# nianticlabs/mickey

Measured on AMD Instinct MI355X. Metric: image pairs/sec (540x720), higher is better.
Workload: dtype bf16

## Files before the change

include/mickey_hip_dev.h:

```cpp
#ifndef MICKEY_HIP_DEV_H
#define MICKEY_HIP_DEV_H

#ifdef __cplusplus
extern "C" {
#endif

int mk_gemm_set_tile(int mode);

int mk_attn_set_mode(int mode);

int mk_dev_mfma_sustained(float* scratch, int workgroups, int iters, int zero_operands, void* stream);

#ifdef __cplusplus
}
#endif
#endif
```

mickey_amd/_native.py:

```python
import ctypes
import os

import torch

from . import build as _build

MK_BF16, MK_F16, MK_F32 = 0, 1, 2
ACT_NONE, ACT_RELU, ACT_GELU = 0, 1, 2

_P, _I, _L, _F, _U = ctypes.c_void_p, ctypes.c_int, ctypes.c_longlong, ctypes.c_float, ctypes.c_ulonglong
_CODES = {"p": _P, "i": _I, "l": _L, "f": _F, "u": _U}

SIGNATURES = {
    "mk_version": ("i", ""),
    "mk_last_error": ("s", ""),
    "mk_preprocess_u8": ("i", "pliiipiip"),
    "mk_gemm": ("i", "pipippiiiiiiip"),
    "mk_gemm_grouped": ("i", "pilpilplpiliiiiiiip"),
    "mk_gemm_ls_residual": ("i", "pipipppiiiiip"),
    "mk_gemm_qkv": ("i", "pipippppiiiifip"),
    "mk_gemm_patch_embed": ("i", "pipipppiiiiip"),
    "mk_gemm_ls_residual_ln": ("i", "pipippppipppiiiiip"),
    "mk_gemm_patch_embed_ln": ("i", "pipipppppiiiiip"),
    "mk_cls_token_ln": ("i", "pppppiiiip"),
# ... 20 lines not shown
    "mk_conv_train_weight_planes": ("i", "piiippppp"),
    "mk_conv_wgrad_work_floats": ("l", "iiiii"),
    "mk_conv_wgrad": ("i", "ppippiiiiippppp"),
    "mk_gemm_grouped_split": ("i", "ppilpilplppiliiiiiffpp"),
    "mk_posenc_add": ("i", "ppppiiiiiip"),
    "mk_linattn_work_floats": ("l", "iiii"),
    "mk_linattn_kv": ("i", "pppiiiip"),
    "mk_linattn_apply": ("i", "pppiiiiiip"),
    "mk_linattn_kv_fused": ("i", "pilpilppiiiiip"),
    "mk_linattn_apply_fused": ("i", "pilpilppilppfpiliiiiip"),
    "mk_linattn_train_work_floats": ("l", "iiii"),
    "mk_linattn_train_fwd": ("i", "pllpllpllfpppiiiip"),
    "mk_linattn_train_bwd": ("i", "pllpllpllppfpppppiiiip"),
    "mk_train_rows_per_chunk": ("i", "i"),
    "mk_train_chunks": ("i", "i"),
    "mk_train_ln_steps": ("i", "i"),
    "mk_train_linear_fwd": ("i", "pliplipppipliiip"),
    "mk_train_linear_ln128_fwd": ("i", "pliplipppfplpppip"),
    "mk_train_linear_dgrad": ("i", "pllipppiplplipliiiip"),
    "mk_train_linear_wgrad": ("i", "pllipliplipliiiip"),
    "mk_train_tail": ("i", "plilplilpp"),
    "mk_train_ln128_fwd": ("i", "pppfplpppip"),
    "mk_train_ln128_bwd": ("i", "pppppplip"),
    "mk_train_headtail_chunk_rows": ("i", ""),
    "mk_train_headtail_chunks": ("i", "l"),
    "mk_train_headtail_fwd": ("i", "pppiiiiiififfp"),
    "mk_train_headtail_bwd": ("i", "ppppppppiiiiiffp"),
    "mk_train_desc_l2norm_fwd": ("i", "pppiiifp"),
    "mk_train_desc_l2norm_bwd": ("i", "ppppiiip"),
    "mk_train_bn_chunk_rows": ("i", ""),
    "mk_train_bn_chunks": ("i", "l"),
    "mk_train_bn_work_floats": ("l", "li"),
    "mk_train_bn_fwd": ("i", "plppplpppffpplpppiiiip"),
    "mk_train_bn_bwd": ("i", "plplpppppplplppfiiip"),
    "mk_optim_chunk_elems": ("i", ""),
    "mk_optim_chunks": ("l", "l"),
    "mk_optim_grad_stats": ("i", "pipipp"),
    "mk_optim_reduce": ("i", "pifpp"),
    "mk_optim_adam": ("i", "pipipp"),
    "mk_head_tails": ("i", "pppppppppppiiiiiiiififp"),
    "mk_dual_softmax_work_floats": ("l", "iiii"),
    "mk_dual_softmax": ("i", "ppppfifppppiiiip"),
    "mk_dual_softmax_split_work_floats": ("l", "iii"),
    "mk_dual_softmax_split": ("i", "ppppfifppppiiiip"),
    "mk_sinkhorn_work_floats": ("l", "iii"),
    "mk_sinkhorn": ("i", "ppppfippppiiiip"),
    "mk_dual_softmax_kf": ("i", "ppppfifppppiiiipip"),
    "mk_dual_softmax_split_kf": ("i", "ppppfifppppiiiipip"),
    "mk_sinkhorn_kf": ("i", "ppppfippppiiiipip"),
    "mk_dual_softmax_pairs": ("i", "ppppfifppppiiiippiip"),
    "mk_dual_softmax_split_pairs_work_floats": ("l", "iiiiii"),
    "mk_dual_softmax_split_pairs": ("i", "ppppfifppppiiiippiip"),
    "mk_sinkhorn_pairs": ("i", "ppppfippppiiiippiip"),
    "mk_dsc_split_planes_floats": ("l", "ii"),
    "mk_dsc_split_planes": ("i", "ppiiip"),
    "mk_dual_softmax_split_planes_work_floats": ("l", "iii"),
    "mk_dual_softmax_split_planes": ("i", "ppppfifppppiiippiip"),
    "mk_mutual_nn": ("i", "ppppiiip"),
    "mk_dual_softmax_train_work_floats": ("l", "iiii"),
    "mk_dual_softmax_train": ("i", "ppppfppppppiiiiip"),
    "mk_dual_softmax_bwd_work_floats": ("l", "iiii"),
    "mk_dual_softmax_bwd": ("i", "ppppfpppppppppiiiiip"),
    "mk_exprace_topk_work_bytes": ("l", "iiil"),
    "mk_exprace_topk_state_bytes": ("l", "ii"),
    "mk_exprace_topk": ("i", "ppuupppppiiliip"),
    "mk_counter_add": ("i", "pup"),
    "mk_gather_backproject": ("i", "ppppppppppppiiiiip"),
    "mk_gather_backproject_kf": ("i", "ppppppppppppiiiiipip"),
    "mk_gather_backproject_pairs": ("i", "ppppppppppppiiiiippiip"),
    "mk_gather_backproject_bwd": ("i", "ppppppppppiiiiip"),
    "mk_ransac_hypotheses": ("i", "pppppuupfppppiiilp"),
    "mk_refine_pose": ("i", "pppppfiipppppppiiiip"),
    "mk_pose_finalize": ("i", "ppppip"),
    "mk_train_ransac_masks": ("i", "pppppuupfiipppiiilp"),
    "mk_reinforce_scatter": ("i", "ppppiiilp"),
    "mk_train_tail_fwd": ("i", "pppppppiiiifiifpppp"),
    "mk_train_tail_bwd": ("i", "pppppppiiiifiifppppppp"),
    "mk_train_aggregate_fwd": ("i", "pppiiififfppppp"),
    "mk_train_aggregate_bwd": ("i", "ppiiipp"),
}

DEV_SIGNATURES = {
    "mk_gemm_set_tile": ("i", "i"),
    "mk_attn_set_mode": ("i", "i"),
    "mk_dev_mfma_sustained": ("i", "piiip"),
}

_lib = None
_missing = set()


class MickeyHipError(RuntimeError):
    pass


def lib_path():
    return os.environ.get("MICKEY_HIP_LIB", _build.lib_path())


def load():
    global _lib
    if _lib is not None:
        return _lib
    path = lib_path()
    if not os.path.exists(path):
        raise MickeyHipError("libmickey_hip.so not found at %s -- build it with `python -m mickey_amd.build` "
                             "(mickey_amd has no CPU/ATen fallback)" % path)
    lib = ctypes.CDLL(path)
    for name, (res, args) in list(SIGNATURES.items()) + list(DEV_SIGNATURES.items()):
        try:
            fn = getattr(lib, name)
        except AttributeError:
            _missing.add(name)
            continue
        fn.restype = ctypes.c_char_p if res == "s" else _CODES[res]
        fn.argtypes = [_CODES[c] for c in args]
    _lib = lib
    return lib


def exported_symbols():
    return list(SIGNATURES)


def missing_symbols():
    load()
    return sorted(_missing)


def ptr(t):
    if t is None:
        return None
    if not t.is_cuda:
        raise MickeyHipError("expected a device tensor")
    return t.data_ptr()


def stream():
    return torch.cuda.current_stream().cuda_stream


def dtype_code(dt):
    if dt == torch.bfloat16:
        return MK_BF16
    if dt == torch.float16:
        return MK_F16
    if dt == torch.float32:
        return MK_F32
    raise MickeyHipError("unsupported low-precision dtype %s" % dt)


def call(name, *args):
    lib = load()
    if name in _missing:
        raise MickeyHipError("libmickey_hip.so does not export %s (stale build?)" % name)
    rc = getattr(lib, name)(*args)
    if rc != 0:
        raise MickeyHipError("%s failed (%d): %s" % (name, rc, lib.mk_last_error().decode()))


def query(name, *args):
    return getattr(load(), name)(*args)
```

mickey_amd/csrc/mk_gemm.hip:

```cpp
#include "mk_gemm_common.hpp"

namespace mk {
namespace gemm {
namespace {

template <typename T, int AMODE, int WMF, bool SP = false>
__global__ __launch_bounds__(256, 1) void gemm_kernel(GemmParams p) {
  using V8 = typename Lp<T>::V8;
  constexpr int NWM = 2, NWN = 2;
  constexpr int NW = NWM * NWN, BM = NWM * WMF * 16, BN = NWN * 64;
  constexpr int AJ = BM / 8 / NW, WJ = BN / 8 / NW;
  constexpr int A_BYTES = BM * 128, STAGE_BYTES = (BM + BN) * 128;
  constexpr int NS = WMF == 2 ? 3 : 2;
  constexpr int PIECES = AJ + WJ;
  extern __shared__ __attribute__((aligned(16))) char smem[];

  const int tid = threadIdx.x;
  const int lane = tid & 63;
  const int wave = __builtin_amdgcn_readfirstlane(tid >> 6);
  const int wm = wave / NWN, wn = wave % NWN;
  const int g = blockIdx.y;
  const int ntm = (p.M + BM - 1) / BM, ntn = (p.N + BN - 1) / BN;
  const int nk = p.K / BK;
  const int fr = lane & 15, fg = lane >> 4;

  const int id = xcd_remap(blockIdx.x, ntm * ntn);
  const int m0 = (id / ntn) * BM, n0 = (id % ntn) * BN;
  Stager<T, AMODE, NW, AJ, WJ, SP> st;
  st.init(p, g, m0, n0, wave, lane);
  st.issue(p, smem, smem + A_BYTES, 0);
  if (NS == 3 && nk > 1) st.issue(p, smem + STAGE_BYTES, smem + STAGE_BYTES + A_BYTES, 1);
  float2* lnp = (float2*)(smem + NS * STAGE_BYTES);
  if (AMODE == A_DENSE && p.ln_stats && tid < 2 * BM) ln_params_to_lds<BM, 2 * BM>(p, m0, tid, lnp, p.ln_shift_out != nullptr && n0 == 0);
  f32x4 acc[WMF][4];
#pragma unroll
  for (int i = 0; i < WMF; ++i)
#pragma unroll
    for (int j = 0; j < 4; ++j) acc[i][j] = f32x4{0.f, 0.f, 0.f, 0.f};
  int cur = 0, nxt = NS - 1;
  for (int kt = 0; kt < nk; ++kt) {
    if (NS == 3 && kt + 1 < nk) asm volatile("s_waitcnt vmcnt(%0)" ::"n"(PIECES) : "memory");
    else asm volatile("s_waitcnt vmcnt(0)" ::: "memory");
    asm volatile("s_waitcnt lgkmcnt(0)" ::: "memory");
    __builtin_amdgcn_s_barrier();
    char* nA = smem + nxt * STAGE_BYTES;
    if (kt + NS - 1 < nk) st.issue(p, nA, nA + A_BYTES, kt + NS - 1);
    const char* sA = smem + cur * STAGE_BYTES;
    const char* sW = sA + A_BYTES;
    cur = cur + 1 == NS ? 0 : cur + 1;
    nxt = nxt + 1 == NS ? 0 : nxt + 1;
    if constexpr (SP) {
      V8 wf[2][4], xf[2][WMF];
#pragma unroll
      for (int ks = 0; ks < 2; ++ks) {
#pragma unroll
        for (int i = 0; i < 4; ++i) {
          const int rw = wn * 64 + i * 16 + fr;
          wf[ks][i] = *(const V8*)(sW + rw * 128 + swz8(rw, ks * 4 + fg) * 16);
        }
#pragma unroll
        for (int i = 0; i < WMF; ++i) {
          const int rx = wm * (WMF * 16) + i * 16 + fr;
          xf[ks][i] = *(const V8*)(sA + rx * 128 + swz8(rx, ks * 4 + fg) * 16);
        }
      }
#pragma unroll
      for (int pr = 0; pr < 3; ++pr) {
        if (pr == 2 && p.npass == 2) break;
#pragma unroll
        for (int mi = 0; mi < WMF; ++mi)
#pragma unroll
          for (int ni = 0; ni < 4; ++ni) acc[mi][ni] = Lp<T>::mma16(wf[pr == 1][ni], xf[pr == 2][mi], acc[mi][ni]);
      }
    } else {
#pragma unroll
      for (int ks = 0; ks < 2; ++ks) {
        V8 wf[4], xf[WMF];
#pragma unroll
        for (int i = 0; i < 4; ++i) {
          const int rw = wn * 64 + i * 16 + fr;
          wf[i] = *(const V8*)(sW + rw * 128 + swz8(rw, ks * 4 + fg) * 16);
        }
#pragma unroll
        for (int i = 0; i < WMF; ++i) {
          const int rx = wm * (WMF * 16) + i * 16 + fr;
          xf[i] = *(const V8*)(sA + rx * 128 + swz8(rx, ks * 4 + fg) * 16);
        }
#pragma unroll
        for (int mi = 0; mi < WMF; ++mi)
#pragma unroll
          for (int ni = 0; ni < 4; ++ni) acc[mi][ni] = Lp<T>::mma16(wf[ni], xf[mi], acc[mi][ni]);
      }
    }
  }
  epilogue<T, WMF>(p, acc, m0, n0, wm, wn, lane, g, lnp);
}

template <typename T, int AMODE, int WMF, bool SP = false>
int launch_small(const GemmParams& p, int groups, hipStream_t st) {
  constexpr int BM = 32 * WMF;
  constexpr int LDS = (WMF == 2 ? 3 : 2) * (BM + 128) * 128 + BM * 8;
  static bool attr_done = false;
  if (!attr_done) {
    hipError_t e = hipFuncSetAttribute((const void*)gemm_kernel<T, AMODE, WMF, SP>, hipFuncAttributeMaxDynamicSharedMemorySize, LDS);
    if (e != hipSuccess) {
      mk_set_error("gemm: cannot reserve %d B of LDS: %s", LDS, hipGetErrorString(e));
      return MK_ERR_LAUNCH;
    }
    attr_done = true;
  }
  const int ntm = (p.M + BM - 1) / BM, ntn = (p.N + 127) / 128;
  hipLaunchKernelGGL((gemm_kernel<T, AMODE, WMF, SP>), dim3(ntm * ntn, groups, 1), dim3(256), LDS, st, p);
  MK_CHECK_LAUNCH();
  return MK_OK;
}

int g_num_cus = 0;
int g_band_m = 0;
int g_half_rows = 1;
int g_schedule = 0;

template <int AMODE>
int launch(const GemmParams& p, int groups, int dtype, hipStream_t st) {
  const long long big_tiles = (long long)((p.M + 255) / 256) * ((p.N + 255) / 256) * groups;
  bool big = p.N >= 256 && big_tiles >= 192;
  const long long plmax = p.npass > 1 ? (long long)max(max(p.pl1[0], p.pl1[1]), max(p.pl2[0], p.pl2[1])) / 2 : 0;
  const bool k_ok = p.K >= 2 * BK && (long long)p.M * p.lda + plmax < (1ll << 31) && (long long)p.N * p.ldw < (1ll << 31) &&
                    (AMODE == A_DENSE || bordered_rows(p.M / (p.H * p.Wd), p.H, p.Wd) * (p.C1 > p.C2 ? p.C1 : p.C2) + plmax < (1ll << 31));
  const bool ln_fold = p.ln_stats || p.xh;
  if (dtype == MK_F32) {
    MK_CHECK_ARG(!ln_fold, "gemm: the folded-LayerNorm epilogues exist for 16-bit operands only");
    return launch_f32(p, groups, AMODE, st);
  }
  int sched = g_schedule;
  if (sched == 0) sched = (big && k_ok) ? 7 : 1;
  if (!k_ok) sched = 1;
  if (sched == 7) return launch_pp64(p, groups, dtype, AMODE, st, g_band_m);
  const long long small_tiles = (long long)((p.M + 127) / 128) * ((p.N + 127) / 128) * groups;
  const bool half_rows = g_schedule == 2 || (g_schedule != 1 && g_half_rows && small_tiles < 2 * num_cus() && p.M > 64);
  if (p.npass > 1)
    return half_rows ? launch_small<_Float16, AMODE, 2, true>(p, groups, st) : launch_small<_Float16, AMODE, 4, true>(p, groups, st);
  if (half_rows) return dtype == MK_BF16 ? launch_small<__bf16, AMODE, 2>(p, groups, st) : launch_small<_Float16, AMODE, 2>(p, groups, st);
  return dtype == MK_BF16 ? launch_small<__bf16, AMODE, 4>(p, groups, st) : launch_small<_Float16, AMODE, 4>(p, groups, st);
}

int check_common(const GemmParams& p, int dtype) {
  MK_CHECK_ARG(dtype == MK_BF16 || dtype == MK_F16 || dtype == MK_F32, "gemm: dtype must be MK_BF16, MK_F16 or MK_F32");
  MK_CHECK_ARG(p.M > 0 && p.N > 0 && p.K > 0, "gemm: empty problem M=%d N=%d K=%d", p.M, p.N, p.K);
  const int kt = dtype == MK_F32 ? KT<float> : BK;
  MK_CHECK_ARG(p.K % kt == 0, "gemm: K=%d must be a multiple of %d", p.K, kt);
  MK_CHECK_ARG(p.N % 4 == 0, "gemm: N=%d must be a multiple of 4", p.N);
  MK_CHECK_ARG(p.ldw % 8 == 0 && p.ldw >= p.K, "gemm: ldw=%d must be >= K and a multiple of 8", p.ldw);
  MK_CHECK_ARG(p.A && p.W, "gemm: null operand");
  return MK_OK;
}

}

int num_cus() {
  if (g_num_cus == 0) {
    int dev = 0, n = 0;
    if (hipGetDevice(&dev) != hipSuccess || hipDeviceGetAttribute(&n, hipDeviceAttributeMultiprocessorCount, dev) != hipSuccess || n <= 0)
      n = 256;
    g_num_cus = n;
  }
  return g_num_cus;
}

}
}

using namespace mk;
using namespace mk::gemm;

extern "C" {

int mk_gemm_set_tile(int mode) {
  if (mode >= 400 && mode < 464) {
    g_band_m = mode - 400;
    return MK_OK;
  }
  if (mode >= 464 && mode < 496) {
    g_band_m = -(mode - 464);
    return MK_OK;
  }
  if (mode == 500 || mode == 501) {
    g_half_rows = mode - 500;
    return MK_OK;
  }
  if (mode >= 600 && mode <= 602) {
    g_pp64_persist = mode - 600;
    return MK_OK;
  }
  MK_CHECK_ARG(mode == 0 || mode == 1 || mode == 2 || mode == 7,
               "mk_gemm_set_tile: unknown mode %d (0 automatic, 1 128x128, 2 64x128, 7 8-wave ping-pong)", mode);
  g_schedule = mode;
  return MK_OK;
}

int mk_gemm(const void* A, int lda, const void* W, int ldw, const float* bias, void* out, int ldc, int M, int N, int K,
            int act, int out_is_f32, int dtype, mk_stream_t stream) {
  GemmParams p = {};
  p.A = A; p.W = W; p.M = M; p.N = N; p.K = K; p.lda = lda; p.ldw = ldw;
  p.epi = MK_EPI_STORE; p.act = act; p.bias = bias; p.ldc = ldc;
  if (out_is_f32) p.out_f32 = (float*)out; else p.out_lp = out;
  if (int e = check_common(p, dtype)) return e;
  MK_CHECK_ARG(lda % 8 == 0 && lda >= K && ldc % 4 == 0 && ldc >= N && out, "mk_gemm: bad lda/ldc/out");
  return launch<A_DENSE>(p, 1, dtype, (hipStream_t)stream);
}

int mk_gemm_grouped(const void* A, int lda, long long strideA, const void* W, int ldw, long long strideW, const float* bias,
                    long long strideBias, void* out, int ldc, long long strideOut, int groups, int M, int N, int K, int act,
                    int out_is_f32, int dtype, mk_stream_t stream) {
  GemmParams p = {};
  p.A = A; p.W = W; p.M = M; p.N = N; p.K = K; p.lda = lda; p.ldw = ldw;
  p.strideA_g = strideA; p.strideW_g = strideW; p.strideBias_g = strideBias; p.strideOut_g = strideOut;
  p.epi = MK_EPI_STORE; p.act = act; p.bias = bias; p.ldc = ldc;
  if (out_is_f32) p.out_f32 = (float*)out; else p.out_lp = out;
  if (int e = check_common(p, dtype)) return e;
  MK_CHECK_ARG(groups > 0 && lda % 8 == 0 && lda >= K && ldc % 4 == 0 && ldc >= N && out, "mk_gemm_grouped: bad args");
  return launch<A_DENSE>(p, groups, dtype, (hipStream_t)stream);
}

int mk_gemm_ls_residual(const void* A, int lda, const void* W, int ldw, const float* bias, const float* gamma, float* x,
                        int ldx, int M, int N, int K, int dtype, mk_stream_t stream) {
  GemmParams p = {};
  p.A = A; p.W = W; p.M = M; p.N = N; p.K = K; p.lda = lda; p.ldw = ldw;
  p.epi = MK_EPI_LS_RESIDUAL; p.bias = bias; p.gamma = gamma; p.out_f32 = x; p.ldc = ldx;
  if (int e = check_common(p, dtype)) return e;
  MK_CHECK_ARG(bias && gamma && x && lda % 8 == 0 && lda >= K && ldx % 4 == 0 && ldx >= N, "mk_gemm_ls_residual: bad args");
  return launch<A_DENSE>(p, 1, dtype, (hipStream_t)stream);
}

int mk_gemm_qkv(const void* A, int lda, const void* W, int ldw, const float* bias, void* q, void* k, void* vt, int nimg,
                int ntok, int ntok_pad, int heads, float qscale, int dtype, mk_stream_t stream) {
  GemmParams p = {};
  const int D = heads * 64;
  p.A = A; p.W = W; p.M = nimg * ntok; p.N = 3 * D; p.K = D; p.lda = lda; p.ldw = ldw;
  p.epi = MK_EPI_QKV; p.bias = bias; p.q = q; p.k = k; p.vt = vt;
  p.ntok = ntok; p.ntok_pad = ntok_pad; p.heads = heads; p.qscale = qscale;
  if (int e = check_common(p, dtype)) return e;
  MK_CHECK_ARG(bias && q && k && vt && ntok_pad % 64 == 0 && ntok_pad >= ntok && lda % 8 == 0 && lda >= D, "mk_gemm_qkv: bad args");
  return launch<A_DENSE>(p, 1, dtype, (hipStream_t)stream);
}

int mk_gemm_patch_embed(const void* A, int lda, const void* W, int ldw, const float* bias, const float* pos, float* x,
                        int nimg, int npatch, int D, int K, int dtype, mk_stream_t stream) {
  GemmParams p = {};
  p.A = A; p.W = W; p.M = nimg * npatch; p.N = D; p.K = K; p.lda = lda; p.ldw = ldw;
  p.epi = MK_EPI_PATCH; p.bias = bias; p.pos = pos; p.npatch = npatch; p.out_f32 = x; p.ldc = D;
  if (int e = check_common(p, dtype)) return e;
  MK_CHECK_ARG(bias && pos && x && lda % 8 == 0 && lda >= K, "mk_gemm_patch_embed: bad args");
  return launch<A_DENSE>(p, 1, dtype, (hipStream_t)stream);
}


static int ln_consumer_args(GemmParams& p, const float* colsum, const float* stats, float eps, float* shift_out, const char* who) {
  MK_CHECK_ARG(colsum && stats && p.bias, "%s: colsum, stats and bias are required", who);
  MK_CHECK_ARG(p.lda == p.K, "%s: the normalised width is K: lda must equal K", who);
  p.ln_colsum = colsum; p.ln_stats = stats; p.ln_nslot = p.K / 64; p.ln_eps = eps; p.ln_shift_out = shift_out;
  return MK_OK;
}

int mk_gemm_ln(const void* A, int lda, const void* W, int ldw, const float* bias, const float* colsum, const float* stats,
               float eps, float* shift_out, void* out, int ldc, int M, int N, int K, int act, int dtype, mk_stream_t stream) {
  GemmParams p = {};
  p.A = A; p.W = W; p.M = M; p.N = N; p.K = K; p.lda = lda; p.ldw = ldw;
  p.epi = MK_EPI_STORE; p.act = act; p.bias = bias; p.ldc = ldc; p.out_lp = out;
  if (int e = check_common(p, dtype)) return e;
  MK_CHECK_ARG(lda % 8 == 0 && ldc % 4 == 0 && ldc >= N && out && (act == MK_ACT_NONE || act == MK_ACT_GELU), "mk_gemm_ln: bad args");
  if (int e = ln_consumer_args(p, colsum, stats, eps, shift_out, "mk_gemm_ln")) return e;
  return launch<A_DENSE>(p, 1, dtype, (hipStream_t)stream);
}

int mk_gemm_qkv_ln(const void* A, int lda, const void* W, int ldw, const float* bias, const float* colsum, const float* stats,
                   float eps, float* shift_out, void* q, void* k, void* vt, int nimg, int ntok, int ntok_pad, int heads,
                   float qscale, int dtype, mk_stream_t stream) {
  GemmParams p = {};
  const int D = heads * 64;
// ... 146 lines not shown
```

mickey_amd/csrc/mk_gemm_common.hpp:

```cpp
#pragma once
#include "mk_common.hpp"

namespace mk {
namespace gemm {

constexpr int BK = 64;
template <typename T> constexpr int EPC = 16 / (int)sizeof(T);
template <typename T> constexpr int KT = 128 / (int)sizeof(T);

enum AMode { A_DENSE = 0, A_CONV3 = 1 };

struct GemmParams {
  const void* A;
  const void* A2;
  const void* W;
  int M, N, K, lda, ldw;
  long long strideA_g, strideA2_g, strideW_g;
  int H, Wd, C1, C2;
  int bord_out;
  unsigned pl1[2], pl2[2];
  int npass;
  float acc_scale;
  void* out_lo;
  float plane_scale;
  int* sat_flag;
  int epi;
  int act;
  const float* bias;
  const float* gamma;
  long long strideBias_g;
  float* out_f32;
  void* out_lp;
  int ldc;
  long long strideOut_g;
  const void* resid_lp;
  long long strideResid_g;
  void* q;
  void* k;
  void* vt;
  int ntok, ntok_pad, heads;
  float qscale;
  const float* pos;
  int npatch;
  void* xh;
  void* xl;
  int ldxs;
  float* stats_out;
  int nslot_out;
  const float* ln_stats;
  const float* ln_colsum;
  int ln_nslot;
  float ln_eps;
  float* ln_shift_out;
  const float* ln_shift_in;
};

__device__ __forceinline__ void quad_stats(const f32x4& x, float& s, float& q) {
  s = x[0];
  s += x[1];
  s += x[2];
  s += x[3];
  q = __builtin_fmaf(x[0], x[0], 0.0f);
  q = __builtin_fmaf(x[1], x[1], q);
  q = __builtin_fmaf(x[2], x[2], q);
  q = __builtin_fmaf(x[3], x[3], q);
}

__device__ __forceinline__ float row16_sum(float v) {
#define MK_DPP_ADD(ctrl) v += __builtin_bit_cast(float, __builtin_amdgcn_update_dpp(0, __builtin_bit_cast(int, v), ctrl, 0xf, 0xf, true))
  MK_DPP_ADD(0xB1);
  MK_DPP_ADD(0x4E);
  MK_DPP_ADD(0x141);
  MK_DPP_ADD(0x140);
#undef MK_DPP_ADD
  return v;
}

typedef __attribute__((ext_vector_type(4))) unsigned u32x4;
struct LnRowLoads16 {
  u32x4 v[4];
  __device__ __forceinline__ void issue(const GemmParams& p, int m0, int tid) {
    const int wave = tid >> 6, lane = tid & 63;
    const long long last = (long long)p.M * 128 - 16;
#pragma unroll
    for (int j = 0; j < 4; ++j) {
      long long off = ((long long)(m0 + wave * 32 + j * 8) * 128) + lane * 16;
      off = off < last ? off : last;
      const char* a = (const char*)p.ln_stats + off;
      asm volatile("global_load_dwordx4 %0, %1, off" : "=v"(v[j]) : "v"(a) : "memory");
    }
  }
  template <int YOUNGER>
  __device__ __forceinline__ void finish(const GemmParams& p, int tid, float2* prm, int m0 = 0, bool publish = false) {
    asm volatile("s_waitcnt vmcnt(%4)" : "+v"(v[0]), "+v"(v[1]), "+v"(v[2]), "+v"(v[3]) : "n"(YOUNGER) : "memory");
    const int wave = tid >> 6, lane = tid & 63;
#pragma unroll
    for (int j = 0; j < 4; ++j) {
      const f32x4 f = __builtin_bit_cast(f32x4, v[j]);
      float s = f[0] + f[2], q = f[1] + f[3];
#define MK_DPP_ADD(x, ctrl) x += __builtin_bit_cast(float, __builtin_amdgcn_update_dpp(0, __builtin_bit_cast(int, x), ctrl, 0xf, 0xf, true))
      MK_DPP_ADD(s, 0xB1);  MK_DPP_ADD(q, 0xB1);
      MK_DPP_ADD(s, 0x4E);  MK_DPP_ADD(q, 0x4E);
      MK_DPP_ADD(s, 0x141); MK_DPP_ADD(q, 0x141);
#undef MK_DPP_ADD
      const double mean = (double)s * (1.0 / 1024.0);
      double var = (double)q * (1.0 / 1024.0) - mean * mean;
      var = var > 0.0 ? var : 0.0;
      const float rstd = 1.0f / sqrtf((float)var + p.ln_eps);
      if ((lane & 7) == 0) {
        const int r = wave * 32 + j * 8 + (lane >> 3);
        prm[r] = make_float2(rstd, -(float)mean * rstd);
        if (publish && m0 + r < p.M) p.ln_shift_out[m0 + r] = (float)mean;
      }
    }
  }
};

struct LnRowDma16 {
  template <int J0>
  __device__ __forceinline__ static void issue(const GemmParams& p, int m0, int wave, int lane, char* stage_lds) {
    const long long last = (long long)p.M * 128 - 16;
#pragma unroll
    for (int j = J0; j < J0 + 2; ++j) {
      const long long base = (long long)(m0 + wave * 32 + j * 8) * 128;
      long long off = base + lane * 16;
      off = off < last ? off : last;
      glds16_sv((const char*)p.ln_stats, (unsigned)off, stage_lds + (wave * 2 + (j - J0)) * 1024);
    }
  }
  template <int J0>
  __device__ __forceinline__ static void finish(const GemmParams& p, int wave, int lane, float2* prm, const char* stage_lds, int m0,
                                                bool publish) {
#pragma unroll
    for (int j = J0; j < J0 + 2; ++j) {
      const f32x4 f = *(const f32x4*)(stage_lds + (wave * 2 + (j - J0)) * 1024 + lane * 16);
      float s = f[0] + f[2], q = f[1] + f[3];
#define MK_DPP_ADD(x, ctrl) x += __builtin_bit_cast(float, __builtin_amdgcn_update_dpp(0, __builtin_bit_cast(int, x), ctrl, 0xf, 0xf, true))
// ... 762 lines not shown
```

mickey_amd/csrc/mk_gemm_pp64.hip:

```cpp
#include <type_traits>

#include "mk_gemm_common.hpp"

namespace mk {
namespace gemm {
int g_pp64_persist = 2;
namespace {

template <typename T, int AMODE, int KIND, bool PERSIST = false, bool SP = false, bool SP2 = false>
__global__ __launch_bounds__(512, 2) void gemm_pp64_kernel(GemmParams p, int band_m) {
  static_assert(!SP2 || SP, "SP2 is a form of the split-operand kernel");
  static_assert(!PERSIST || AMODE == A_DENSE, "the persistent tile loop is built for dense operands");
  static_assert(!SP || (KIND == 0 && !PERSIST && sizeof(T) == 2), "split operands: plain epilogues, one tile per workgroup");
  constexpr int BKA = SP ? BK / 2 : BK;
  using V8 = typename Lp<T>::V8;
  constexpr int WMF = 8, BM = 256, BN = 256;
  constexpr int A_BYTES = BM * 128, STAGE_BYTES = (BM + BN) * 128;
  constexpr int LN_STAGE_OFF = 2 * STAGE_BYTES + 256 * 8;
  extern __shared__ __attribute__((aligned(16))) char smem[];

  const int tid0 = threadIdx.x;
  const int wave = __builtin_amdgcn_readfirstlane(tid0 >> 6);
  int lane = tid0 & 63, tid = tid0;
  auto refresh_lane = [&]() {
    if constexpr (PERSIST) {
      asm volatile("v_mbcnt_lo_u32_b32 %0, -1, 0\n\tv_mbcnt_hi_u32_b32 %0, -1, %0" : "=v"(lane));
      tid = wave * 64 + lane;
    }
  };
  const int wm = wave >> 2, wn = wave & 3;
  const int g = blockIdx.y;
  const int ntm = (p.M + BM - 1) / BM, ntn = (p.N + BN - 1) / BN;
  const int nk = p.K / BK;

  const T* A = (const T*)p.A + (long long)g * p.strideA_g;
  const T* A2 = p.A2 ? (const T*)p.A2 + (long long)g * p.strideA2_g : nullptr;
  const T* W = (const T*)p.W + (long long)g * p.strideW_g;
  int srow = lane >> 3, sp = lane & 7;
  const int ntiles = ntm * ntn;
  auto tile_origin = [&](int id, int& mm, int& nn) {
    int tm, tn;
    pp_tile_coords(xcd_remap(id, ntiles), ntm, ntn, band_m, tm, tn);
    mm = tm * BM;
    nn = tn * BN;
  };
  int bid = blockIdx.x;
  int m0, n0;
  tile_origin(bid, m0, n0);
  unsigned woff[4], aoff[4], aoff2[4];
  auto set_woff = [&](int nn0) {
#pragma unroll
    for (int j = 0; j < 4; ++j) {
      const int rw = (wave * 4 + j) * 8 + srow;
      int n = nn0 + rw;
      n = n < p.N ? n : p.N - 1;
      woff[j] = ((unsigned)n * (unsigned)p.ldw + swz8(rw, sp) * 8) * (unsigned)sizeof(T);
    }
  };
  auto set_aoff = [&](int mm0) {
#pragma unroll
    for (int j = 0; j < 4; ++j) {
      const int ra = wm * 128 + (wn * 4 + j) * 8 + srow;
      int m = mm0 + ra;
      m = m < p.M ? m : p.M - 1;
      const int c = swz8(ra, sp);
      const unsigned cc = SP ? (unsigned)(c & 3) : (unsigned)c;
      const bool lo = SP && (c >> 2) != 0;
      const unsigned pb1 = !SP ? 0u : (lo ? p.pl1[1] : p.pl1[0]), pb2 = !SP ? 0u : (lo ? p.pl2[1] : p.pl2[0]);
      if (AMODE == A_DENSE) {
        aoff[j] = ((unsigned)m * (unsigned)p.lda + cc * 8) * (unsigned)sizeof(T) + pb1;
        aoff2[j] = 0;
      } else {
        const unsigned br = (unsigned)bordered_row(m, p.H, p.Wd);
        aoff[j] = (br * (unsigned)p.C1 + cc * 8) * (unsigned)sizeof(T) + pb1;
        aoff2[j] = (br * (unsigned)p.C2 + cc * 8) * (unsigned)sizeof(T) + pb2;
      }
    }
  };
  set_woff(n0);
  set_aoff(m0);
  auto dma_w1 = [&](int s, int j) {
    glds16_sv(W + s * BK, woff[j], smem + (s & 1) * STAGE_BYTES + A_BYTES + (wave * 4 + j) * 1024);
  };
  const int ntap = A2 ? 10 : 9;
  const T* cbase = AMODE == A_DENSE ? A : A - (long long)(p.Wd + 2) * p.C1;
  int cleft = p.C1, ctap = 0;
  auto conv_advance = [&]() {
    cleft -= BKA;
    const bool wrap = cleft == 0;
    ctap += wrap ? 1 : 0;
    const int ty = (ctap * 11) >> 5, tx = ctap - 3 * ty;
    const T* tapbase = ctap < 9 ? A + (long long)((ty - 1) * (p.Wd + 1) + tx - 1) * p.C1 : A2;
    cbase = wrap ? tapbase : cbase + BKA;
    cleft = wrap ? (ctap < 9 ? p.C1 : p.C2) : cleft;
  };
  auto dma_a1 = [&](int s, int j) {
    char* dst = smem + (s & 1) * STAGE_BYTES + (wm * 16 + wn * 4 + j) * 1024;
    if (AMODE == A_DENSE) {
      glds16_sv(A + s * BKA, aoff[j], dst);
    } else {
      glds16_sv(cbase, ctap < 9 ? aoff[j] : aoff2[j], dst);
    }
  };
  auto dma_w = [&](int s) {
#pragma unroll
    for (int j = 0; j < 4; ++j) dma_w1(s, j);
  };
  auto dma_a = [&](int s) {
#pragma unroll
    for (int j = 0; j < 4; ++j) dma_a1(s, j);
    if (AMODE != A_DENSE) conv_advance();
  };

  int fr = lane & 15, fg = lane >> 4;
  auto derive_lane = [&]() {
    srow = lane >> 3;
    sp = lane & 7;
    fr = lane & 15;
    fg = lane >> 4;
  };
  auto load_w = [&](V8* wf, int par, int h) {
    const char* sW = smem + par * STAGE_BYTES + A_BYTES;
#pragma unroll
    for (int i = 0; i < 4; ++i) {
      const int rw = wn * 64 + i * 16 + fr;
      wf[i] = *(const V8*)(sW + rw * 128 + swz8(rw, h * 4 + fg) * 16);
// ... 192 lines not shown
      }
    };
    auto second_stage_done = [&]() {
      if constexpr (PERSIST) {
        if (ln_pending && ln_fast)
          LnRowDma16::finish<2>(p, wave, lane, (float2*)(smem + 2 * STAGE_BYTES), smem + LN_STAGE_OFF, m0,
                                ln && p.ln_shift_out != nullptr && n0 == 0);
      }
    };
    ln_pending = PERSIST && bid != (int)blockIdx.x;
    int kt0 = 0;
    if (wm == 0) {
      if constexpr (PERSIST) {
        stage0(0, Yes{}, Yes{}, 1, 2, Yes{});
        first_stage_done();
        stage0(1, Yes{}, Yes{}, 2, 3, No{});
        second_stage_done();
        kt0 = 2;
      }
      for (int kt = kt0; kt < nk - 2; ++kt) stage0(kt, Yes{}, Yes{}, kt + 1, kt + 2, No{});
      if constexpr (PERSIST) {
        set_aoff(m1);
        stage0(nk - 2, Yes{}, Yes{}, nk - 1, 0, No{});
        set_woff(n1);
        stage0(nk - 1, Yes{}, No{}, 0, 0, No{});
      } else {
        stage0(nk - 2, Yes{}, No{}, nk - 1, 0, No{});
        stage0(nk - 1, No{}, No{}, 0, 0, No{});
      }
      bar();
    } else {
      bar();
      if constexpr (PERSIST) {
        stage1(0, Yes{}, Yes{}, 1, 2, Yes{});
        first_stage_done();
        stage1(1, Yes{}, Yes{}, 2, 3, No{});
        second_stage_done();
        kt0 = 2;
      }
      for (int kt = kt0; kt < nk - 2; ++kt) stage1(kt, Yes{}, Yes{}, kt + 1, kt + 2, No{});
      if constexpr (PERSIST) {
        set_aoff(m1);
        stage1(nk - 2, Yes{}, Yes{}, nk - 1, 0, No{});
        set_woff(n1);
        stage1(nk - 1, Yes{}, No{}, 0, 0, No{});
      } else {
        stage1(nk - 2, Yes{}, No{}, nk - 1, 0, No{});
        stage1(nk - 1, No{}, No{}, 0, 0, No{});
      }
    }
    char* wl0 = smem + STAGE_BYTES + wave * 4096;
    refresh_lane();
    epilogue_lds<T, KIND, AMODE == A_CONV3>(p, acc, wl0, wl0 + A_BYTES, m0, n0, wm, wn, lane, g, (const float2*)(smem + 2 * STAGE_BYTES));
    if (!(PERSIST && has_next)) break;
    bid = nbid;
    m0 = m1;
    n0 = n1;
    asm volatile("" : "+s"(m0), "+s"(n0));
    refresh_lane();
    if (ln_fast) LnRowDma16::issue<0>(p, m0, wave, lane, smem + LN_STAGE_OFF);
    if constexpr (PRODUCER) shl.issue(p, m0, tid, 256);
  }
}

template <typename T, int AMODE, int KIND, bool PERSIST, bool SP = false, bool SP2 = false>
int launch_k2(const GemmParams& p, int groups, hipStream_t st, int band_m, int grid) {
  constexpr int LDS = 2 * 512 * 128 + 256 * 8 + (PERSIST && KIND == 1 ? 16384 : 0);
  static bool attr_done = false;
  if (!attr_done) {
    hipError_t e = hipFuncSetAttribute((const void*)gemm_pp64_kernel<T, AMODE, KIND, PERSIST, SP, SP2>, hipFuncAttributeMaxDynamicSharedMemorySize, LDS);
    if (e != hipSuccess) {
      mk_set_error("gemm: cannot reserve %d B of LDS: %s", LDS, hipGetErrorString(e));
      return MK_ERR_LAUNCH;
    }
    attr_done = true;
  }
  hipLaunchKernelGGL((gemm_pp64_kernel<T, AMODE, KIND, PERSIST, SP, SP2>), dim3(grid, groups, 1), dim3(512), LDS, st, p, band_m);
  MK_CHECK_LAUNCH();
  return MK_OK;
}

template <typename T, int AMODE, int KIND>
int launch_k(const GemmParams& p, int groups, hipStream_t st, int band_m) {
  const int ntm = (p.M + 255) / 256, ntn = (p.N + 255) / 256;
  if (band_m == 0) band_m = (AMODE == A_DENSE && ntn <= 4) ? -4 : 8;
  if constexpr (KIND == 0 && sizeof(T) == 2 && std::is_same<T, _Float16>::value) {
    if (p.npass == 2) {
      if constexpr (AMODE == A_CONV3) return launch_k2<T, AMODE, 0, false, true, true>(p, groups, st, band_m, ntm * ntn);
    }
    if (p.npass > 1) return launch_k2<T, AMODE, 0, false, true>(p, groups, st, band_m, ntm * ntn);
  }
  if constexpr (AMODE == A_DENSE && KIND != 0) {
    const int nk = p.K / BK, grid = num_cus() & ~7;
    const bool ok = groups == 1 && p.npass <= 1 && (nk & 1) == 0 && nk >= 4 && grid >= 8 && ntm * ntn > grid &&
                    !(KIND == 1 && p.ln_stats && p.ln_nslot != 16);
    if (g_pp64_persist != 1 && ok && !(g_pp64_persist == 2 && KIND == 1)) return launch_k2<T, AMODE, KIND, true>(p, groups, st, band_m, grid);
  }
  return launch_k2<T, AMODE, KIND, false>(p, groups, st, band_m, ntm * ntn);
}

template <typename T>
int launch_dense(const GemmParams& p, int groups, hipStream_t st, int band_m) {
  if (p.xh && p.epi == MK_EPI_LS_RESIDUAL && p.out_f32) return launch_k<T, A_DENSE, 3>(p, groups, st, band_m);
  if (p.xh) return launch_k<T, A_DENSE, 2>(p, groups, st, band_m);
  if (p.ln_stats) return launch_k<T, A_DENSE, 1>(p, groups, st, band_m);
  return launch_k<T, A_DENSE, 0>(p, groups, st, band_m);
}

}

int launch_pp64(const GemmParams& p, int groups, int dtype, int amode, hipStream_t st, int band_m) {
  if (amode == A_DENSE) return dtype == MK_BF16 ? launch_dense<__bf16>(p, groups, st, band_m) : launch_dense<_Float16>(p, groups, st, band_m);
  return dtype == MK_BF16 ? launch_k<__bf16, A_CONV3, 0>(p, groups, st, band_m) : launch_k<_Float16, A_CONV3, 0>(p, groups, st, band_m);
}

}
}
```

mickey_amd/ops.py:

```python

import numpy as np
import torch


from ._native import ACT_GELU, ACT_NONE, ACT_RELU, call, dtype_code, ptr, query, stream

LOG2E = 1.4426950408889634


def _chk(t, dtype=None):
    assert t.is_cuda and t.is_contiguous(), "expected a contiguous device tensor"
    if dtype is not None:
        assert t.dtype == dtype, "expected %s, got %s" % (dtype, t.dtype)
    return t


def preprocess_u8(frames, H, W, out=None):
    assert frames.is_cuda and frames.dtype == torch.uint8 and frames.dim() == 4 and frames.shape[3] == 3 and frames.is_contiguous()
    n, Hs, Ws, _ = frames.shape
    if out is None:
        out = torch.empty((n, 3, H, W), device=frames.device, dtype=torch.float32)
    call("mk_preprocess_u8", ptr(frames), Hs * Ws * 3, n, Hs, Ws, ptr(out), H, W, stream())
    return out


def gemm_set_tile(mode):
    call("mk_gemm_set_tile", int(mode))


def gemm(a, w, bias=None, act=ACT_NONE, out_f32=False, out=None, lda=None, K=None):
    M = a.shape[0]
    lda = a.shape[1] if lda is None else lda
    N, ldw = w.shape
    K = min(lda, ldw) if K is None else K
    if out is None:
        out = torch.empty((M, N), device=a.device, dtype=torch.float32 if out_f32 else a.dtype)
    call("mk_gemm", ptr(a), lda, ptr(w), ldw, ptr(bias), ptr(out), out.stride(0), M, N, K, act,
         int(out.dtype == torch.float32), dtype_code(a.dtype), stream())
    return out


def gemm_grouped(a, w, bias, out, groups, M, N, K, lda, ldw, ldc, stride_a, stride_w, stride_bias, stride_out, act=ACT_NONE):
    call("mk_gemm_grouped", ptr(a), lda, stride_a, ptr(w), ldw, stride_w, ptr(bias), stride_bias, ptr(out), ldc, stride_out,
         groups, M, N, K, act, int(out.dtype == torch.float32), dtype_code(a.dtype), stream())
    return out


def gemm_ls_residual(a, w, bias, gamma, x):
    M, K = a.shape
    N = w.shape[0]
    call("mk_gemm_ls_residual", ptr(a), a.stride(0), ptr(w), w.stride(0), ptr(bias), ptr(gamma), ptr(x), x.stride(0), M, N, K,
         dtype_code(a.dtype), stream())
    return x


def gemm_qkv(a, w, bias, q, k, vt, nimg, ntok, ntok_pad, heads):
    qscale = (64.0 ** -0.5) * LOG2E
    call("mk_gemm_qkv", ptr(a), a.stride(0), ptr(w), w.stride(0), ptr(bias), ptr(q), ptr(k), ptr(vt), nimg, ntok, ntok_pad,
         heads, qscale, dtype_code(a.dtype), stream())


def gemm_ls_residual_ln(a, w, bias, gamma, xh, xl, stats, x_out=None, shift=None):
    M, K = a.shape
    N = w.shape[0]
    call("mk_gemm_ls_residual_ln", ptr(a), a.stride(0), ptr(w), w.stride(0), ptr(bias), ptr(gamma), ptr(xh), ptr(xl),
         xh.stride(0), ptr(stats), ptr(shift), ptr(x_out), x_out.stride(0) if x_out is not None else N, M, N, K,
         dtype_code(a.dtype), stream())


def gemm_patch_embed_ln(a, w, bias, pos, xh, xl, stats, nimg, npatch):
    D = w.shape[0]
    call("mk_gemm_patch_embed_ln", ptr(a), a.stride(0), ptr(w), w.stride(0), ptr(bias), ptr(pos), ptr(xh), ptr(xl), ptr(stats),
         nimg, npatch, D, w.shape[1], dtype_code(a.dtype), stream())


def cls_token_ln(cls, pos, xh, xl, stats, nimg, ntok, D):
    call("mk_cls_token_ln", ptr(cls), ptr(pos), ptr(xh), ptr(xl), ptr(stats), nimg, ntok, D, dtype_code(xh.dtype), stream())


def recentre_split(xh, xl, stats):
    rows, D = xh.shape
    call("mk_recentre_split", ptr(xh), ptr(xl), ptr(stats), rows, D, dtype_code(xh.dtype), stream())


def gemm_ln(a, w, bias, colsum, stats, eps, act=ACT_NONE, out=None, shift_out=None):
    M, K = a.shape
    N = w.shape[0]
    if out is None:
        out = torch.empty((M, N), device=a.device, dtype=a.dtype)
    call("mk_gemm_ln", ptr(a), a.stride(0), ptr(w), w.stride(0), ptr(bias), ptr(colsum), ptr(stats), float(eps), ptr(shift_out),
         ptr(out), out.stride(0), M, N, K, act, dtype_code(a.dtype), stream())
    return out


def gemm_qkv_ln(a, w, bias, colsum, stats, eps, q, k, vt, nimg, ntok, ntok_pad, heads, shift_out=None):
    qscale = (64.0 ** -0.5) * LOG2E
    call("mk_gemm_qkv_ln", ptr(a), a.stride(0), ptr(w), w.stride(0), ptr(bias), ptr(colsum), ptr(stats), float(eps),
         ptr(shift_out), ptr(q), ptr(k), ptr(vt), nimg, ntok, ntok_pad, heads, qscale, dtype_code(a.dtype), stream())


def im2col_patch14(img, gh, gw, ldo, dtype, out=None):
    assert img.dtype == torch.float32 and img.stride(3) == 1
    nimg = img.shape[0]
    if out is None:
        out = torch.empty((nimg * gh * gw, ldo), device=img.device, dtype=dtype)
    assert out.shape == (nimg * gh * gw, ldo) and out.dtype == dtype and out.is_contiguous()
    call("mk_im2col_patch14", ptr(img), img.stride(0), img.stride(1), img.stride(2), nimg, gh, gw, ptr(out), ldo,
         dtype_code(dtype), stream())
    return out

# ... 915 lines not shown
```

Before: 281.2.

## Split big GEMM into full-wave ping-pong head and small-tile tail launch

When the 256x256 ping-pong GEMM leaves a partial last wave of tiles, a cost model splits the M dimension. Full rounds of tiles run with the big kernel, and the leftover rows run as a second launch with 128- or 64-row tiles. New tm_base/ntm_sub fields let the kernels cover a sub-range of M-tiles. The aim is to cut wave-quantization idle time, at the cost of an extra kernel launch and a heuristic whose constants may misjudge some shapes.

```diff
diff --git a/include/mickey_hip_dev.h b/include/mickey_hip_dev.h
--- a/include/mickey_hip_dev.h
+++ b/include/mickey_hip_dev.h
@@ -7,6 +7,8 @@
 
 int mk_gemm_set_tile(int mode);
 
+int mk_gemm_last_split(int* head_mtiles, int* tail_form);
+
 int mk_attn_set_mode(int mode);
 
 int mk_dev_mfma_sustained(float* scratch, int workgroups, int iters, int zero_operands, void* stream);
diff --git a/mickey_amd/_native.py b/mickey_amd/_native.py
--- a/mickey_amd/_native.py
+++ b/mickey_amd/_native.py
@@ -126,6 +126,7 @@
 
 DEV_SIGNATURES = {
     "mk_gemm_set_tile": ("i", "i"),
+    "mk_gemm_last_split": ("i", "pp"),
     "mk_attn_set_mode": ("i", "i"),
     "mk_dev_mfma_sustained": ("i", "piiip"),
 }
diff --git a/mickey_amd/csrc/mk_gemm.hip b/mickey_amd/csrc/mk_gemm.hip
--- a/mickey_amd/csrc/mk_gemm.hip
+++ b/mickey_amd/csrc/mk_gemm.hip
@@ -20,12 +20,12 @@
   const int wave = __builtin_amdgcn_readfirstlane(tid >> 6);
   const int wm = wave / NWN, wn = wave % NWN;
   const int g = blockIdx.y;
-  const int ntm = (p.M + BM - 1) / BM, ntn = (p.N + BN - 1) / BN;
+  const int ntm = p.ntm_sub ? p.ntm_sub : (p.M + BM - 1) / BM, ntn = (p.N + BN - 1) / BN;
   const int nk = p.K / BK;
   const int fr = lane & 15, fg = lane >> 4;
 
   const int id = xcd_remap(blockIdx.x, ntm * ntn);
-  const int m0 = (id / ntn) * BM, n0 = (id % ntn) * BN;
+  const int m0 = (p.tm_base + id / ntn) * BM, n0 = (id % ntn) * BN;
   Stager<T, AMODE, NW, AJ, WJ, SP> st;
   st.init(p, g, m0, n0, wave, lane);
   st.issue(p, smem, smem + A_BYTES, 0);
@@ -109,7 +109,7 @@
     }
     attr_done = true;
   }
-  const int ntm = (p.M + BM - 1) / BM, ntn = (p.N + 127) / 128;
+  const int ntm = p.ntm_sub ? p.ntm_sub : (p.M + BM - 1) / BM, ntn = (p.N + 127) / 128;
   hipLaunchKernelGGL((gemm_kernel<T, AMODE, WMF, SP>), dim3(ntm * ntn, groups, 1), dim3(256), LDS, st, p);
   MK_CHECK_LAUNCH();
   return MK_OK;
@@ -120,8 +120,48 @@
 int g_half_rows = 1;
 int g_schedule = 0;
 
+int g_tail_split = 0;
+int g_last_head = 0, g_last_tail = 0;
+constexpr float TS_PP_US = 1.75f;
+constexpr float TS_US[3] = {0.f, 1.4f, 1.0f};
+constexpr float TS_LAUNCH_US = 20.0f;
+constexpr float TS_MARGIN = 0.10f;
+constexpr int TS_MIN_HEAD_ROUNDS = 4;
+
+inline int tail_split_plan(const GemmParams& p, int groups, int& head_m) {
+  head_m = 0;
+  if (g_tail_split == 1 || p.npass > 1) return 0;
+  if (p.ln_stats) return 0;
+  const long long ntm = (p.M + 255) / 256, ntn = (p.N + 255) / 256, per_m = ntn * groups, tiles = ntm * per_m;
+  const int cus = num_cus();
+  const long long rounds = tiles / cus;
+  const bool pinned = g_tail_split == 2 || g_tail_split == 3;
+  if (rounds < (pinned ? 1 : TS_MIN_HEAD_ROUNDS) || per_m > cus) return 0;
+  const long long hm = rounds * cus / per_m;
+  if (hm <= 0 || hm >= ntm) return 0;
+  const long long tail_rows = p.M - hm * 256;
+  const float nk = (float)(p.K / BK);
+  const float keep = ((float)((tiles + cus - 1) / cus) - (float)(hm * per_m) / (float)cus) * nk * TS_PP_US;
+  const long long ntn_s = (p.N + 127) / 128;
+  float cost[3] = {keep, 0.f, 0.f};
+  for (int f = 1; f <= 2; ++f) {
+    const int bm = f == 1 ? 128 : 64;
+    const long long n = ((tail_rows + bm - 1) / bm) * ntn_s * groups;
+    cost[f] = (float)((n + 2 * cus - 1) / (2 * cus)) * nk * TS_US[f] + TS_LAUNCH_US;
+  }
+  int best = cost[2] < cost[1] ? 2 : 1;
+  if (pinned) best = g_tail_split - 1;
+  else if (!(cost[best] < keep * (1.f - TS_MARGIN))) return 0;
+  head_m = (int)hm;
+  return best;
+}
+
+template <int AMODE>
+int launch_small_form(const GemmParams& p, int groups, int dtype, hipStream_t st, bool half_rows);
+
 template <int AMODE>
 int launch(const GemmParams& p, int groups, int dtype, hipStream_t st) {
+  g_last_head = g_last_tail = 0;
   const long long big_tiles = (long long)((p.M + 255) / 256) * ((p.N + 255) / 256) * groups;
   bool big = p.N >= 256 && big_tiles >= 192;
   const long long plmax = p.npass > 1 ? (long long)max(max(p.pl1[0], p.pl1[1]), max(p.pl2[0], p.pl2[1])) / 2 : 0;
@@ -135,9 +175,28 @@
   int sched = g_schedule;
   if (sched == 0) sched = (big && k_ok) ? 7 : 1;
   if (!k_ok) sched = 1;
-  if (sched == 7) return launch_pp64(p, groups, dtype, AMODE, st, g_band_m);
+  if (sched == 7) {
+    int head_m = 0;
+    const int tail = g_schedule == 0 ? tail_split_plan(p, groups, head_m) : 0;
+    if (!tail) return launch_pp64(p, groups, dtype, AMODE, st, g_band_m);
+    GemmParams h = p, t = p;
+    h.tm_base = 0;
+    h.ntm_sub = head_m;
+    if (int e = launch_pp64(h, groups, dtype, AMODE, st, g_band_m)) return e;
+    const int bm = tail == 1 ? 128 : 64;
+    t.tm_base = head_m * (256 / bm);
+    t.ntm_sub = (p.M - head_m * 256 + bm - 1) / bm;
+    g_last_head = head_m;
+    g_last_tail = tail;
+    return launch_small_form<AMODE>(t, groups, dtype, st, tail == 2);
+  }
   const long long small_tiles = (long long)((p.M + 127) / 128) * ((p.N + 127) / 128) * groups;
   const bool half_rows = g_schedule == 2 || (g_schedule != 1 && g_half_rows && small_tiles < 2 * num_cus() && p.M > 64);
+  return launch_small_form<AMODE>(p, groups, dtype, st, half_rows);
+}
+
+template <int AMODE>
+int launch_small_form(const GemmParams& p, int groups, int dtype, hipStream_t st, bool half_rows) {
   if (p.npass > 1)
     return half_rows ? launch_small<_Float16, AMODE, 2, true>(p, groups, st) : launch_small<_Float16, AMODE, 4, true>(p, groups, st);
   if (half_rows) return dtype == MK_BF16 ? launch_small<__bf16, AMODE, 2>(p, groups, st) : launch_small<_Float16, AMODE, 2>(p, groups, st);
@@ -192,9 +251,20 @@
     g_pp64_persist = mode - 600;
     return MK_OK;
   }
+  if (mode >= 700 && mode <= 703) {
+    g_tail_split = mode - 700;
+    return MK_OK;
+  }
   MK_CHECK_ARG(mode == 0 || mode == 1 || mode == 2 || mode == 7,
                "mk_gemm_set_tile: unknown mode %d (0 automatic, 1 128x128, 2 64x128, 7 8-wave ping-pong)", mode);
   g_schedule = mode;
+  return MK_OK;
+}
+
+int mk_gemm_last_split(int* head_mtiles, int* tail_form) {
+  MK_CHECK_ARG(head_mtiles && tail_form, "mk_gemm_last_split: null argument");
+  *head_mtiles = g_last_head;
+  *tail_form = g_last_tail;
   return MK_OK;
 }
 
diff --git a/mickey_amd/csrc/mk_gemm_common.hpp b/mickey_amd/csrc/mk_gemm_common.hpp
--- a/mickey_amd/csrc/mk_gemm_common.hpp
+++ b/mickey_amd/csrc/mk_gemm_common.hpp
@@ -53,6 +53,7 @@
   float ln_eps;
   float* ln_shift_out;
   const float* ln_shift_in;
+  int tm_base, ntm_sub;
 };
 
 __device__ __forceinline__ void quad_stats(const f32x4& x, float& s, float& q) {
diff --git a/mickey_amd/csrc/mk_gemm_pp64.hip b/mickey_amd/csrc/mk_gemm_pp64.hip
--- a/mickey_amd/csrc/mk_gemm_pp64.hip
+++ b/mickey_amd/csrc/mk_gemm_pp64.hip
@@ -30,7 +30,7 @@
   };
   const int wm = wave >> 2, wn = wave & 3;
   const int g = blockIdx.y;
-  const int ntm = (p.M + BM - 1) / BM, ntn = (p.N + BN - 1) / BN;
+  const int ntm = p.ntm_sub ? p.ntm_sub : (p.M + BM - 1) / BM, ntn = (p.N + BN - 1) / BN;
   const int nk = p.K / BK;
 
   const T* A = (const T*)p.A + (long long)g * p.strideA_g;
@@ -41,7 +41,7 @@
   auto tile_origin = [&](int id, int& mm, int& nn) {
     int tm, tn;
     pp_tile_coords(xcd_remap(id, ntiles), ntm, ntn, band_m, tm, tn);
-    mm = tm * BM;
+    mm = (p.tm_base + tm) * BM;
     nn = tn * BN;
   };
   int bid = blockIdx.x;
@@ -400,7 +400,7 @@
 
 template <typename T, int AMODE, int KIND>
 int launch_k(const GemmParams& p, int groups, hipStream_t st, int band_m) {
-  const int ntm = (p.M + 255) / 256, ntn = (p.N + 255) / 256;
+  const int ntm = p.ntm_sub ? p.ntm_sub : (p.M + 255) / 256, ntn = (p.N + 255) / 256;
   if (band_m == 0) band_m = (AMODE == A_DENSE && ntn <= 4) ? -4 : 8;
   if constexpr (KIND == 0 && sizeof(T) == 2 && std::is_same<T, _Float16>::value) {
     if (p.npass == 2) {
diff --git a/mickey_amd/ops.py b/mickey_amd/ops.py
--- a/mickey_amd/ops.py
+++ b/mickey_amd/ops.py
@@ -26,6 +26,13 @@
 
 def gemm_set_tile(mode):
     call("mk_gemm_set_tile", int(mode))
+
+
+def gemm_last_split():
+    import ctypes
+    head, tail = ctypes.c_int(0), ctypes.c_int(0)
+    call("mk_gemm_last_split", ctypes.addressof(head), ctypes.addressof(tail))
+    return head.value, tail.value
 
 
 def gemm(a, w, bias=None, act=ACT_NONE, out_f32=False, out=None, lda=None, K=None):
```

After: 281.5, median of 2. About the same (+0.1%).
